# xingchensong/TouchNet

Hardware: AMD Instinct MI355X
Metric: audio+text tokens/sec/node (packed seq, full train step) + step MFU (higher is better)
Workload: dtype bf16

## Files before the change

### include/touchnet_amd.h

```cpp
#ifndef TOUCHNET_AMD_H_
#define TOUCHNET_AMD_H_

#ifdef __cplusplus
extern "C" {
#endif

const char* tn_version(void);

int tn_norm_bwd_workspace_floats(int rows, int H);
int tn_rmsnorm_fwd(const void* x, const void* res_in, const void* w, void* y, void* res_out, float* rstd,
                   int rows, int H, float eps, int dtype, void* stream);
int tn_rmsnorm_bwd(const void* dy, const void* h, const void* w, const float* rstd, const void* dres, void* dh,
                   void* dw, float* workspace, int rows, int H, int dtype, void* stream);

int tn_layernorm_fwd(const void* x, const void* res_in, const void* w, const void* b, void* y, void* res_out,
                     float* mean, float* rstd, int rows, int H, float eps, int dtype, void* stream);
int tn_layernorm_bwd(const void* dy, const void* h, const void* w, const float* mean, const float* rstd,
                     const void* dres, void* dh, void* dw, void* db, float* workspace, int rows, int H, int dtype,
                     void* stream);

int tn_swiglu_fwd(const void* gate, const void* up, void* out, long long n, int dtype, void* stream);
int tn_swiglu_bwd(const void* dout, const void* gate, const void* up, void* dgate, void* dup, long long n,
                  int dtype, void* stream);
int tn_swiglu_fwd_t(const void* gate, const void* up, void* out, void* out_t, int rows, int cols, void* stream);
// ... 79 lines not shown
int tn_transpose_bf16(const void* src, void* dst, int rows, int cols, long long src_ld, long long dst_ld,
                      void* stream);

long long tn_colsum_workspace_floats(int rows, int cols);
int tn_colsum_bf16(const void* x, void* out, float* ws, int rows, int cols, long long ld, void* stream);

int tn_pcm16_to_f32(const void* pcm_int16, float* out, long long n, void* stream);

int tn_bestrq_tokenize(const float* feat, const float* quantizer, const float* codebook, long long* codes, int T,
                       int F, int E, int V, void* stream);

int tn_pack_plan(const int* lens, int n, int B, int T, int skip_too_long, int* row, int* col, int* sent, int* batch,
                 int* counts, void* stream);
int tn_pack_fill(const int* row, const int* col, const int* sent, const int* batch, int which_batch, int n,
                 const int* ntok, const long long* tok_off, const long long* tokens, const int* alen,
                 const long long* feat_off, const float* feat_src, int F, int B, int T, long long bos, long long eos,
                 long long pad, long long* input_ids, long long* labels, long long* position_ids, long long* doc,
                 long long* sentence_lens, float* feats, int* nsent, void* stream);

int tn_gemm_bf16(const void* const* A, const void* const* B, const long long* lda, const long long* ldb, const int* K,
                 int nseg, int a_kmaj, int b_kmaj, void* C, void* Ct, const void* bias, int M, int N, long long ldc,
                 long long ldct, int accumulate, void* stream);
int tn_gemm_bf16_addend(const void* A, const void* B, long long lda, long long ldb, int K, int a_kmaj, int b_kmaj, void* C,
                        const void* bias, const void* addend, long long ldadd, int M, int N, long long ldc, void* stream);
int tn_gemm_bf16_splitk(const void* A, const void* B, long long lda, long long ldb, int K, int a_kmaj, int b_kmaj,
                        void* C, const void* bias, int M, int N, long long ldc, int accumulate, int splitk, int tail_only,
                        void* workspace, long long workspace_bytes, void* stream);
int tn_gemm_bf16_wgrad_f32(const void* A, const void* B, long long lda, long long ldb, int K, float* C, int M, int N,
                           long long ldc, int accumulate, int splitk, void* workspace, long long workspace_bytes,
                           void* stream);
int tn_gemm_bf16_wgrad_bias(const void* A, const void* B, long long lda, long long ldb, int K, void* C, void* bias_grad,
                            int M, int N, long long ldc, int accumulate, int c_f32, int splitk, void* workspace,
                            long long workspace_bytes, void* stream);
long long tn_gemm_grouped_workspace_bytes(const int* M, const int* N, const int* K, int ngrp);
int tn_gemm_bf16_grouped(const void* const* A, const void* const* B, const long long* lda, const long long* ldb,
                         const int* K, void* const* C, const long long* ldc, const int* M, const int* N, int ngrp,
                         int a_kmaj, int b_kmaj, int accumulate, int c_f32, void* workspace, long long workspace_bytes,
                         void* stream);
int tn_gemm_bf16_swiglu_fwd(const void* x, const void* wg, const void* wu, void* gate, void* up, void* act, int M, int I,
                            int K, long long ldx, long long ldw, long long ldc, void* stream);
int tn_gemm_bf16_swiglu_bwd(const void* dy, const void* wd, const void* gate, const void* up, void* dgate, void* dup,
                            int M, int I, int H, long long lddy, long long ldw, long long ld, void* stream);
int tn_gemm_bf16_gelu_fwd(const void* x, const void* w, const void* bias, void* pre, void* act, int M, int N, int K,
                          long long ldx, long long ldw, long long ldc, void* stream);
int tn_gemm_bf16_gelu_bwd(const void* dy, const void* w2, const void* pre, void* dpre, int M, int I, int H, long long lddy,
                          long long ldw, long long ld, void* stream);
int tn_gemm_bf16_rope(const void* x, const void* w, const void* bias, const void* cos_t, const void* sin_t, void* out, int M,
                      int N, int K, long long ldx, long long ldw, long long ldc, int head_dim, void* stream);
int tn_gemm_bf16_tn(const void* A, const void* B, void* C, void* Ct, const void* bias, int M, int N, int K,
                    long long lda, long long ldb, long long ldc, long long ldct, int accumulate, void* stream);

void tn_gemm_set_persistent(int on);
int tn_gemm_get_persistent(void);

long long tn_attn_decode_workspace_bytes(int B, int Nh, int Nkv, int D, int S_max);
int tn_attn_decode(const void* q, const void* k_new, const void* v_new, void* k_cache, void* v_cache, const int* cache_len,
                   void* o, void* workspace, int B, int Nh, int Nkv, int D, int S_max, float scale, void* stream);
int tn_greedy_step(const void* logits, int* hist, int* hist_len, int* cache_len, int* finished, int* n_unfinished, int B,
                   int V, int S_hist, float penalty, int ngram, int eos, int pad, int dtype, void* stream);
int tn_sample_step(const void* logits, int* hist, int* hist_len, int* cache_len, int* finished, int* n_unfinished,
                   const long long* row_key, const float* uniforms, int* n_kept, int B, int V, int S_hist, float penalty,
                   int do_sample, float temperature, int top_k, float top_p, unsigned long long seed, const int* eos_ids,
                   int n_eos, int pad, int dtype, void* stream);
int tn_kimi_text_step(const void* logits, int* hist, int* hist_len, int* cache_len, int* finished, int* n_unfinished,
                      const int* prompt_len, const void* embed, void* x_next, const long long* row_key,
                      const float* uniforms, int B, int V, int S_hist, int H, float penalty, int window, float temperature,
// ... 21 lines not shown
```

### touchnet_amd/_C.py

```python
from __future__ import annotations

import ctypes as C
import os

import torch

_HERE = os.path.dirname(os.path.abspath(__file__))
LIB_PATH = os.environ.get("TN_AMD_LIB") or os.path.join(_HERE, "_lib", "libtouchnet_amd.so")

_vp, _i, _f, _ll, _ull = C.c_void_p, C.c_int, C.c_float, C.c_longlong, C.c_ulonglong

PROTOTYPES = {
    "tn_version": [],
    "tn_norm_bwd_workspace_floats": [_i, _i],
    "tn_rmsnorm_fwd": [_vp, _vp, _vp, _vp, _vp, _vp, _i, _i, _f, _i, _vp],
    "tn_rmsnorm_bwd": [_vp, _vp, _vp, _vp, _vp, _vp, _vp, _vp, _i, _i, _i, _vp],
    "tn_layernorm_fwd": [_vp, _vp, _vp, _vp, _vp, _vp, _vp, _vp, _i, _i, _f, _i, _vp],
    "tn_layernorm_bwd": [_vp, _vp, _vp, _vp, _vp, _vp, _vp, _vp, _vp, _vp, _i, _i, _i, _vp],
    "tn_swiglu_fwd": [_vp, _vp, _vp, _ll, _i, _vp],
    "tn_swiglu_bwd": [_vp, _vp, _vp, _vp, _vp, _ll, _i, _vp],
    "tn_gelu_fwd": [_vp, _vp, _ll, _i, _vp],
    "tn_gelu_bwd": [_vp, _vp, _vp, _ll, _i, _vp],
    "tn_rope_table": [_vp, _vp, _vp, _vp, _i, _i, _f, _i, _vp],
    "tn_rope_apply": [_vp, _vp, _vp, _vp, _vp, _vp, _i, _i, _i, _i, _i, _i, _vp],
# ... 17 lines not shown
    "tn_log_mel": [_vp, _vp, _vp, _vp, _i, _i, _vp],
    "tn_audiofeat_stack": [_vp, _vp, _i, _i, _i, _i, _i, _vp],
    "tn_resample_polyphase": [_vp, _vp, _vp, _ll, _ll, _i, _i, _i, _vp],
    "tn_feat_augment": [_vp, _vp, _i, _i, _i, _vp, _i, _vp, _i, _vp, _i, _vp],
    "tn_sumsq_scratch_floats": [],
    "tn_sumsq": [_vp, _vp, _vp, _ll, _i, _vp],
    "tn_adamw_step": [_vp, _vp, _vp, _vp, _vp, _vp, _ll, _f, _f, _f, _f, _f, _f, _f, _f, _i, _vp],
    "tn_transpose_bf16": [_vp, _vp, _i, _i, _ll, _ll, _vp],
    "tn_swiglu_fwd_t": [_vp, _vp, _vp, _vp, _i, _i, _vp],
    "tn_swiglu_bwd_t": [_vp, _vp, _vp, _vp, _vp, _vp, _i, _i, _vp],
    "tn_colsum_workspace_floats": [_i, _i],
    "tn_colsum_bf16": [_vp, _vp, _vp, _i, _i, _ll, _vp],
    "tn_pcm16_to_f32": [_vp, _vp, _ll, _vp],
    "tn_bestrq_tokenize": [_vp, _vp, _vp, _vp, _i, _i, _i, _i, _vp],
    "tn_sumsq_multi_chunk": [],
    "tn_sumsq_multi": [_vp, _vp, _vp, _i, _ll, _vp, _vp, _i, _vp],
    "tn_adamw_multi_chunk": [],
    "tn_adamw_prepare": [_vp, _vp, _f, _f, _f, _vp],
    "tn_adamw_multi": [_vp, _vp, _vp, _vp, _vp, _vp, _vp, _i, _ll, _vp, _f, _f, _f, _f, _f, _i, _vp],
    "tn_adamw_multi_bounded": [_vp, _vp, _vp, _vp, _vp, _vp, _vp, _i, _ll, _vp, _f, _f, _f, _f, _f, _i, _i, _vp],
    "tn_pack_plan": [_vp, _i, _i, _i, _i, _vp, _vp, _vp, _vp, _vp, _vp],
    "tn_pack_fill": [_vp, _vp, _vp, _vp, _i, _i, _vp, _vp, _vp, _vp, _vp, _vp, _i, _i, _i, _ll, _ll, _ll, _vp, _vp, _vp,
                     _vp, _vp, _vp, _vp, _vp],
    "tn_gemm_bf16_tn": [_vp, _vp, _vp, _vp, _vp, _i, _i, _i, _ll, _ll, _ll, _ll, _i, _vp],
    "tn_gemm_bf16_addend": [_vp, _vp, _ll, _ll, _i, _i, _i, _vp, _vp, _vp, _ll, _i, _i, _ll, _vp],
    "tn_gemm_bf16_splitk": [_vp, _vp, _ll, _ll, _i, _i, _i, _vp, _vp, _i, _i, _ll, _i, _i, _i, _vp, _ll, _vp],
    "tn_gemm_bf16_wgrad_f32": [_vp, _vp, _ll, _ll, _i, _vp, _i, _i, _ll, _i, _i, _vp, _ll, _vp],
    "tn_gemm_bf16": [C.POINTER(_vp), C.POINTER(_vp), C.POINTER(_ll), C.POINTER(_ll), C.POINTER(_i), _i, _i, _i, _vp, _vp,
                     _vp, _i, _i, _ll, _ll, _i, _vp],
    "tn_gemm_grouped_workspace_bytes": [C.POINTER(_i), C.POINTER(_i), C.POINTER(_i), _i],
    "tn_gemm_bf16_grouped": [C.POINTER(_vp), C.POINTER(_vp), C.POINTER(_ll), C.POINTER(_ll), C.POINTER(_i), C.POINTER(_vp),
                             C.POINTER(_ll), C.POINTER(_i), C.POINTER(_i), _i, _i, _i, _i, _i, _vp, _ll, _vp],
    "tn_gemm_bf16_wgrad_bias": [_vp, _vp, _ll, _ll, _i, _vp, _vp, _i, _i, _ll, _i, _i, _i, _vp, _ll, _vp],
    "tn_gemm_bf16_rope": [_vp, _vp, _vp, _vp, _vp, _vp, _i, _i, _i, _ll, _ll, _ll, _i, _vp],
    "tn_gemm_bf16_gelu_fwd": [_vp, _vp, _vp, _vp, _vp, _i, _i, _i, _ll, _ll, _ll, _vp],
    "tn_gemm_bf16_gelu_bwd": [_vp, _vp, _vp, _vp, _i, _i, _i, _ll, _ll, _ll, _vp],
    "tn_gemm_bf16_swiglu_fwd": [_vp, _vp, _vp, _vp, _vp, _vp, _i, _i, _i, _ll, _ll, _ll, _vp],
    "tn_gemm_bf16_swiglu_bwd": [_vp, _vp, _vp, _vp, _vp, _vp, _i, _i, _i, _ll, _ll, _ll, _vp],
    "tn_gemm_set_persistent": [_i],
    "tn_gemm_get_persistent": [],
    "tn_attn_decode_workspace_bytes": [_i, _i, _i, _i, _i],
    "tn_attn_decode": [_vp, _vp, _vp, _vp, _vp, _vp, _vp, _vp, _i, _i, _i, _i, _i, _f, _vp],
    "tn_greedy_step": [_vp, _vp, _vp, _vp, _vp, _vp, _i, _i, _i, _f, _i, _i, _i, _i, _vp],
    "tn_sample_step": [_vp, _vp, _vp, _vp, _vp, _vp, _vp, _vp, _vp, _i, _i, _i, _f, _i, _f, _i, _f, _ull, _vp, _i, _i, _i,
                       _vp],
    "tn_kimi_text_step": [_vp] * 11 + [_i, _i, _i, _i, _f, _i, _f, _i, _ull, _i, _i, _i, _i, _vp],
    "tn_attn_decode_beam": [_vp, _vp, _vp, _vp, _vp, _vp, _vp, _vp, _vp, _i, _i, _i, _i, _i, _f, _vp],
    "tn_beam_step_workspace_bytes": [_i, _i],
    "tn_beam_step": [_vp] * 17 + [_i, _i, _i, _i, _i, _f, _i, _vp, _i, _i, _f, _i, _i, _vp],
    "tn_attn_block_causal_fwd": [_vp, _vp, _vp, _vp, _vp, _vp, _i, _i, _i, _i, _i, _f, _vp],
    "tn_vq_nearest": [_vp, _vp, _vp, _vp, _i, _i, _i, _vp],
}
_RESTYPE = {"tn_gemm_set_persistent": None, "tn_version": C.c_char_p, "tn_sumsq_multi_chunk": C.c_longlong, "tn_adamw_multi_chunk": C.c_longlong,
            "tn_colsum_workspace_floats": C.c_longlong, "tn_gemm_grouped_workspace_bytes": C.c_longlong,
            "tn_attn_decode_workspace_bytes": C.c_longlong, "tn_beam_step_workspace_bytes": C.c_longlong,
            "tn_philox4x32_10": None}

DEV_PROTOTYPES = {
    "tn_philox4x32_10": [_vp, _ull],
}

_lib = None


class KernelError(RuntimeError):
    pass
# ... 49 lines not shown
```

### touchnet_amd/csrc/gemm.hip

```cpp
#include <stdlib.h>

#include <type_traits>
#include <utility>

#include "common.h"

namespace tn {
namespace gemm {

constexpr int BM = 256, BN = 256;
constexpr int SLOT = 32768;
constexpr int LDS_BYTES = 5 * SLOT;
constexpr int NT = 512;
constexpr int MAXSEG = 3;

typedef __attribute__((address_space(3))) void* lds_ptr_t;
typedef __attribute__((ext_vector_type(2))) uint32_t u32x2_t;
typedef __attribute__((ext_vector_type(4))) uint32_t u32x4_t;

struct Seg {
  const bf16_t* A;
  const bf16_t* B;
  long long lda, ldb;
  int K;
// ... 7 lines not shown
  int start;
  int stages;
};

constexpr int EPI_PLAIN = 0, EPI_GROUPED = 1, EPI_SWIGLU_FWD = 2, EPI_SWIGLU_BWD = 3, EPI_BIASG = 4, EPI_ROPE = 5;
constexpr int EPI_GELU_FWD = 6, EPI_GELU_BWD = 7;

struct Params {
  Seg seg[MAXSEG];
  int nseg;
  int M, N;
  bf16_t* C;
  bf16_t* Ct;
  const bf16_t* bias;
  long long ldc, ldct;
  int accumulate;
  const bf16_t* addend;
  long long ldadd;
  int nbm, nbn;
  int stages;
  int splitk, kchunk;
  float* ws;
  int tile0, ntiles;
  int c_f32;
  Grp grp[MAXSEG];
  int ngrp;
  bf16_t* C2;
  bf16_t* C3;
  const bf16_t* E1;
  const bf16_t* E2;
  long long lde;
  bf16_t* bias_out;
  float* bias_ws;
  const bf16_t* rope_cos;
  const bf16_t* rope_sin;
  int rope_d;
};

__device__ __forceinline__ void tile_of_block(int bid, int nbm, int nbn, int& tm, int& tn) {
  const int total = nbm * nbn;
  const int xcd = bid & 7, local = bid >> 3;
  const int q = total >> 3, r = total & 7;
  const int vid = (xcd < r ? xcd * (q + 1) : r * (q + 1) + (xcd - r) * q) + local;
  constexpr int GM = 8;
  const int per_group = GM * nbn;
  const int g = vid / per_group, w = vid - g * per_group;
  const int gm = min(GM, nbm - g * GM);
  tm = g * GM + w % gm;
  tn = w / gm;
}

typedef f32x16_t Acc[4][2];

constexpr int kPieceB[4] = {0, 2, 4, 6}, kPieceA[4] = {14, 18, 22, 26};
static_assert(kPieceB[3] < kPieceA[0], "every B piece is issued before the first A piece");

template <bool IS_A> constexpr int piece_at(int pos) {
  for (int i = 0; i < 4; ++i)
    if ((IS_A ? kPieceA[i] : kPieceB[i]) == pos) return i;
  return -1;
}
constexpr int early_piece_count() {
  int n = 0;
  for (int i = 0; i < 4; ++i) n += (kPieceB[i] < 8) + (kPieceA[i] < 8);
  return n;
}
// ... 235 lines not shown
    auto zero_acc = [&]() {
#pragma unroll
      for (int i = 0; i < 4; ++i)
#pragma unroll
        for (int j = 0; j < 2; ++j)
#pragma unroll
          for (int r = 0; r < 16; ++r) acc[i][j][r] = 0.f;
    };
    zero_acc();

    Frags<AK, 4> ae, ao;
    Frags<BK, 2> be, bo;

#define TN_PIN() __builtin_amdgcn_sched_barrier(0)
    auto read_frag = [&](auto QC, auto FC, int sa, int sb, Frags<AK, 4>& a, Frags<BK, 2>& b) {
      constexpr int Q = decltype(QC)::value, F = decltype(FC)::value;
      if constexpr (F < 2) rb.template read<Q, F>(smem, sb * SLOT, b);
      else ra.template read<Q, F - 2>(smem, sa * SLOT, a);
    };
    auto read_all = [&](auto QC, int sa, int sb, Frags<AK, 4>& a, Frags<BK, 2>& b) {
      read_frag(QC, std::integral_constant<int, 0>{}, sa, sb, a, b);
      read_frag(QC, std::integral_constant<int, 1>{}, sa, sb, a, b);
      read_frag(QC, std::integral_constant<int, 2>{}, sa, sb, a, b);
      read_frag(QC, std::integral_constant<int, 3>{}, sa, sb, a, b);
      read_frag(QC, std::integral_constant<int, 4>{}, sa, sb, a, b);
      read_frag(QC, std::integral_constant<int, 5>{}, sa, sb, a, b);
    };
    auto mma = [&](const Frags<AK, 4>& a, const Frags<BK, 2>& b, int i, int j) {
      acc[i][j] = __builtin_amdgcn_mfma_f32_32x32x16_bf16(b.v[j], a.v[i], acc[i][j], 0, 0, 0);
    };

    float bsum = 0.f;
    bool bias_on = false;
    auto bias_accum = [&](const Frags<AK, 4>& a) {
      auto add = [&](const bf16x8_t& v) {
        const u32x4_t w = __builtin_bit_cast(u32x4_t, v);
        bsum += ((__uint_as_float(w.x << 16) + __uint_as_float(w.x & 0xffff0000u)) +
                 (__uint_as_float(w.y << 16) + __uint_as_float(w.y & 0xffff0000u))) +
                ((__uint_as_float(w.z << 16) + __uint_as_float(w.z & 0xffff0000u)) +
                 (__uint_as_float(w.w << 16) + __uint_as_float(w.w & 0xffff0000u)));
      };
      if (wc == 0) add(a.v[0]);
      else if (wc == 1) add(a.v[1]);
      else if (wc == 2) add(a.v[2]);
      else add(a.v[3]);
    };

    auto quarter = [&](auto NQC, auto P0C, const Frags<AK, 4>& ca, const Frags<BK, 2>& cb, Frags<AK, 4>& na,
                       Frags<BK, 2>& nb, int nsa, int nsb, int dst_b, int dst_a) {
      constexpr int P0 = decltype(P0C)::value;
      if constexpr (EPI == EPI_BIASG) {
        if (bias_on) bias_accum(ca);
        TN_PIN();
      }
      auto step = [&](auto MC) {
        constexpr int m = decltype(MC)::value;
        mma(ca, cb, m >> 1, m & 1);
        TN_PIN();
        if constexpr (m < 6) {
          read_frag(NQC, std::integral_constant<int, m>{}, nsa, nsb, na, nb);
          TN_PIN();
        }
        constexpr int pb = P0 < 0 ? -1 : piece_at<false>(P0 + m);
        constexpr int pa = P0 < 0 ? -1 : piece_at<true>(P0 + m);
        if constexpr (pb >= 0) {
          piece_b(dst_b, pb);
// ... 32 lines not shown
      one(std::integral_constant<int, 1>{});
      one(std::integral_constant<int, 2>{});
      one(std::integral_constant<int, 3>{});
      one(std::integral_constant<int, 4>{});
      one(std::integral_constant<int, 5>{});
      one(std::integral_constant<int, 6>{});
      one(std::integral_constant<int, 7>{});
    };
    auto next = [](int s, int d) { s += d; return s >= 5 ? s - 5 : s; };
    using I0 = std::integral_constant<int, 0>;
    using I1 = std::integral_constant<int, 1>;
    using I2 = std::integral_constant<int, 2>;
    using I3 = std::integral_constant<int, 3>;
    using NONE = std::integral_constant<int, -1>;

#pragma unroll
    for (int q = 0; q < 4; ++q) piece_a(0, q);
    adv_a();
#pragma unroll
    for (int q = 0; q < 4; ++q) piece_b(1, q);
    adv_b();
#pragma unroll
    for (int q = 0; q < 4; ++q) piece_a(2, q);
    adv_a();
    early_pieces(3, 4);
    asm volatile("s_waitcnt vmcnt(%0)" ::"n"(4 + early_piece_count()) : "memory");
    __builtin_amdgcn_s_barrier();
    int sa = 0, sb = 1;
    int pa = 4, pb = 3;

    auto trip = [&](auto LASTC) {
      constexpr bool LAST = decltype(LASTC)::value;
      const int sa1 = next(sa, 2), sb1 = next(sb, 2);
      __builtin_amdgcn_s_setprio(1);
      quarter(I1{}, std::integral_constant<int, 8>{}, ae, be, ao, bo, sa, sb, pb, pa);
      wait_frags(ao, bo);
      TN_PIN();
      quarter(I2{}, std::integral_constant<int, 16>{}, ao, bo, ae, be, sa, sb, pb, pa);
      wait_frags(ae, be);
      TN_PIN();
      quarter(I3{}, std::integral_constant<int, 24>{}, ae, be, ao, bo, sa, sb, pb, pa);
      __builtin_amdgcn_s_setprio(0);
      wait_frags(ao, bo);
      __builtin_amdgcn_s_waitcnt(0xc07f);
      asm volatile("s_waitcnt vmcnt(4)" ::: "memory");
      __builtin_amdgcn_s_barrier();
      __builtin_amdgcn_s_setprio(1);
      if constexpr (!LAST) {
        quarter(I0{}, I0{}, ao, bo, ae, be, sa1, sb1, sa, sb);
        __builtin_amdgcn_s_setprio(0);
        wait_frags(ae, be);
        TN_PIN();
      } else {
        if constexpr (EPI == EPI_BIASG) {
          if (bias_on) bias_accum(ao);
        }
#pragma unroll
        for (int m = 0; m < 8; ++m) mma(ao, bo, m >> 1, m & 1);
        __builtin_amdgcn_s_setprio(0);
      }
      pb = sa;
      pa = sb;
      sa = sa1;
      sb = sb1;
    };

    const int np_all = SPLITK ? p.kchunk : p.stages;
    for (int kc = 0; kc < mine; ++kc) {
      int np = np_all;
      if constexpr (EPI == EPI_BIASG) {
        int m0_, n0_, g_;
        origin_g(kc, m0_, n0_, g_);
        bias_on = n0_ == 0;
        bsum = 0.f;
      }
      if constexpr (EPI == EPI_GROUPED) {
        int m0_, n0_, g_;
        origin_g(kc, m0_, n0_, g_);
        np = p.grp[g_].stages;
      }
      read_all(I0{}, sa, sb, ae, be);
      wait_frags(ae, be);
      TN_PIN();
      for (int t = 1; t < np; ++t) trip(std::false_type{});
      trip(std::true_type{});
      int m0, n0, grp;
      origin_g(kc, m0, n0, grp);
      if constexpr (EPI == EPI_BIASG) {
        if (bias_on) {
          const float tot = bsum + __shfl_xor(bsum, 32, 64);
          const int m = m0 + wr * 128 + wc * 32 + (lane & 31);
          if (lane < 32) {
            if constexpr (SPLITK) {
              p.bias_ws[(long long)split_of(kc) * (p.nbm * BM) + m] = tot;
            } else if (m < p.M) {
              p.bias_out[m] = f2bf(tot);
            }
          }
        }
      }
      if constexpr (SPLITK) {
        const int u = bid + kc * G, sp = u / tiles;
        epilogue_ws(p, acc, sp * tiles + (u - sp * tiles), wr * 128, wc * 64, lane);
      } else if constexpr (OUT_F32) {
        if constexpr (EPI == EPI_GROUPED) {
          const Out o = {p.grp[grp].C, p.grp[grp].ldc, p.grp[grp].M, p.grp[grp].N};
          epilogue_f32(p, o, acc, m0 + wr * 128, n0 + wc * 64, lane);
        } else {
          const Out o = {p.C, p.ldc, p.M, p.N};
          epilogue_f32(p, o, acc, m0 + wr * 128, n0 + wc * 64, lane);
        }
      } else if constexpr (EPI == EPI_GROUPED) {
        const Out o = {p.grp[grp].C, p.grp[grp].ldc, p.grp[grp].M, p.grp[grp].N};
        epilogue(p, o, acc, smem + (wave < 4 ? pb : pa) * SLOT + (wave & 3) * 8192, m0 + wr * 128, n0 + wc * 64, lane);
      } else {
        const Out o = {p.C, p.ldc, p.M, p.N};
        epilogue(p, o, acc, smem + (wave < 4 ? pb : pa) * SLOT + (wave & 3) * 8192, m0 + wr * 128, n0 + wc * 64, lane);
      }
      zero_acc();
      __builtin_amdgcn_s_waitcnt(0xc07f);
      __builtin_amdgcn_s_barrier();
      asm volatile("" : "+v"(lane));
      ra = Reader<AK, 4>(lane, wr * 128);
      rb = Reader<BK, 2>(lane, wc * 64);
      sA.set_voff(wave, lane);
      sB.set_voff(wave, lane);
      early_pieces(pb, pa);
// ... 765 lines not shown
    float* d = reinterpret_cast<float*>(C) + (long long)m * ldc + n;
    float4 x = make_float4(a[0], a[1], a[2], a[3]), y = make_float4(a[4], a[5], a[6], a[7]);
    if (accumulate) {
      const float4 ox = *reinterpret_cast<const float4*>(d), oy = *reinterpret_cast<const float4*>(d + 4);
      x.x += ox.x; x.y += ox.y; x.z += ox.z; x.w += ox.w;
      y.x += oy.x; y.y += oy.y; y.z += oy.z; y.w += oy.w;
    }
    *reinterpret_cast<float4*>(d) = x;
    *reinterpret_cast<float4*>(d + 4) = y;
    return;
  }
  bf16_t* dst = C + (long long)m * ldc + n;
  if (bias != nullptr) {
    Vec16<bf16_t> b;
    float fb[8];
    b.load(bias + n);
    b.unpack(fb);
#pragma unroll
    for (int e = 0; e < 8; ++e) a[e] += fb[e];
  }
  if (accumulate) {
    Vec16<bf16_t> o;
    float fo[8];
    o.load(dst);
    o.unpack(fo);
#pragma unroll
    for (int e = 0; e < 8; ++e) a[e] += fo[e];
  }
  Vec16<bf16_t> out;
  out.pack(a);
  out.store(dst);
}

template <bool AK, bool BK, bool HAS_CT>
static int launch(dim3 grid, hipStream_t st, const Params& p) {
  constexpr bool WGRAD = AK && BK && !HAS_CT;
  auto reduce = [&](const float* bias_ws, bf16_t* bias_out) {
    hipLaunchKernelGGL(splitk_reduce_kernel, dim3((unsigned)p.ntiles * 32u), dim3(256), 0, st, p.ws, p.splitk, p.M, p.N,
                       p.nbm, p.nbn, p.tile0, p.ntiles, p.C, p.ldc, p.bias, p.accumulate, p.c_f32, bias_ws, bias_out);
  };
  if (p.bias_out != nullptr) {
    if constexpr (WGRAD) {
      if (p.splitk > 1) {
        hipLaunchKernelGGL((gemm_kernel<true, true, false, true, false, EPI_BIASG>), grid, dim3(NT), 0, st, p);
        reduce(p.bias_ws, p.bias_out);
      } else if (p.c_f32) {
        hipLaunchKernelGGL((gemm_kernel<true, true, false, false, true, EPI_BIASG>), grid, dim3(NT), 0, st, p);
      } else {
        hipLaunchKernelGGL((gemm_kernel<true, true, false, false, false, EPI_BIASG>), grid, dim3(NT), 0, st, p);
      }
    } else {
      return -1;
    }
  } else if (p.splitk > 1) {
    if constexpr (!HAS_CT) {
      hipLaunchKernelGGL((gemm_kernel<AK, BK, false, true>), grid, dim3(NT), 0, st, p);
      reduce(nullptr, nullptr);
    } else {
      return -1;
    }
  } else if (p.c_f32) {
    if constexpr (WGRAD) {
      hipLaunchKernelGGL((gemm_kernel<true, true, false, false, true>), grid, dim3(NT), 0, st, p);
    } else {
      return -1;
    }
  } else if constexpr (!AK && !HAS_CT) {
    hipLaunchKernelGGL((gemm16_kernel<AK, BK>), grid, dim3(NT), 0, st, p);
  } else {
    hipLaunchKernelGGL((gemm_kernel<AK, BK, HAS_CT>), grid, dim3(NT), 0, st, p);
  }
  return 0;
}

}
}

extern "C" {

static int g_persistent = 1;
void tn_gemm_set_persistent(int on) { g_persistent = on ? 1 : 0; }
int tn_gemm_get_persistent(void) { return g_persistent; }

// ... 64 lines not shown
  }
  for (int s = nseg; s < MAXSEG; ++s) p.seg[s] = p.seg[0];
  if (Ct != nullptr && ((M % 8) || (ldct % 8) || ldct < M || ((uintptr_t)Ct & 15))) return TN_EINVAL;
  if (Ct != nullptr && accumulate) return TN_EINVAL;
  p.nseg = nseg;
  p.M = M;
  p.N = N;
  p.C = (tn::bf16_t*)C;
  p.Ct = (tn::bf16_t*)Ct;
  p.bias = (const tn::bf16_t*)bias;
  p.ldc = ldc;
  p.ldct = ldct;
  p.accumulate = accumulate;
  p.addend = (const tn::bf16_t*)addend;
  p.ldadd = ldadd;
  p.nbm = (M + BM - 1) / BM;
  p.nbn = (N + BN - 1) / BN;
  p.splitk = 1;
  p.kchunk = 0;
  p.ws = nullptr;
  p.tile0 = 0;
  p.ntiles = p.nbm * p.nbn;
  p.c_f32 = c_f32;
  const int ncu = num_cus();
  int main_tiles = 0;
  if (splitk > 1) {
    if (nseg != 1 || Ct != nullptr) return TN_EINVAL;
    if (!(a_kmaj && b_kmaj) && (p.stages % splitk) != 0) return TN_EINVAL;
    if (tail_only) {
      main_tiles = p.ntiles / ncu * ncu;
      if (main_tiles <= 0 || main_tiles >= p.ntiles) return TN_EINVAL;
    }
    const long long slabs = (long long)splitk * (p.ntiles - main_tiles) * BM * BN;
    if (workspace == nullptr || ((uintptr_t)workspace & 15) ||
        workspace_bytes < (slabs + (bias_grad ? (long long)splitk * p.nbm * BM : 0)) * (long long)sizeof(float))
      return TN_EINVAL;
    p.splitk = splitk;
    p.kchunk = (p.stages + splitk - 1) / splitk;
    p.ws = (float*)workspace;
    p.bias_ws = bias_grad ? (float*)workspace + slabs : nullptr;
  }
  p.bias_out = (tn::bf16_t*)bias_grad;
  const bool persist = persistent_now();
  hipStream_t st = (hipStream_t)stream;
  int rc = 0;
#define TN_MODE(AKM, BKM, GRID, PRM) \
  rc |= (Ct != nullptr) ? launch<AKM, BKM, true>(GRID, st, PRM) : launch<AKM, BKM, false>(GRID, st, PRM)
#define TN_LAUNCH(GRID, PRM)                                                               \
  if (!a_kmaj && !b_kmaj) TN_MODE(false, false, GRID, PRM);                                \
  else if (!a_kmaj && b_kmaj) TN_MODE(false, true, GRID, PRM);                             \
  else if (a_kmaj && b_kmaj) TN_MODE(true, true, GRID, PRM);                               \
  else return TN_EINVAL
  if (main_tiles > 0) {
    Params pm = p;
    pm.splitk = 1;
    pm.ntiles = main_tiles;
    const dim3 gm(ncu);
    TN_LAUNCH(gm, pm);
    p.tile0 = main_tiles;
    p.ntiles -= main_tiles;
  }
  {
    const int units = p.ntiles * p.splitk;
    const dim3 grid(persist && units > ncu ? ncu : units);
    TN_LAUNCH(grid, p);
  }
#undef TN_LAUNCH
#undef TN_MODE
  if (rc != 0) return TN_EINVAL;
  TN_LAUNCH_CHECK();
  return TN_OK;
}

// ... 183 lines not shown
    return TN_EINVAL;
  Params p;
  clear_params(p);
  p.seg[0].A = (const tn::bf16_t*)dy;
  p.seg[0].B = (const tn::bf16_t*)wd;
  p.seg[0].lda = lddy;
  p.seg[0].ldb = ldw;
  p.seg[0].K = H;
  p.seg[1] = p.seg[2] = p.seg[0];
  p.stages = H / 64;
  p.M = M;
  p.N = I;
  p.C = (tn::bf16_t*)dgate;
  p.C2 = (tn::bf16_t*)dup;
  p.E1 = (const tn::bf16_t*)gate;
  p.E2 = (const tn::bf16_t*)up;
  p.ldc = p.lde = ld;
  p.nbm = (M + BM - 1) / BM;
  p.nbn = (I + BN - 1) / BN;
  p.ntiles = p.nbm * p.nbn;
  const int ncu = num_cus();
  const dim3 grid(persistent_now() && p.ntiles > ncu ? ncu : p.ntiles);
  hipLaunchKernelGGL((gemm16_kernel<false, true, EPI_SWIGLU_BWD>), grid, dim3(NT), 0, (hipStream_t)stream, p);
  TN_LAUNCH_CHECK();
  return TN_OK;
}

int tn_gemm_bf16_wgrad_bias(const void* A, const void* B, long long lda, long long ldb, int K, void* C, void* bias_grad,
                            int M, int N, long long ldc, int accumulate, int c_f32, int splitk, void* workspace,
                            long long workspace_bytes, void* stream) {
  if (bias_grad == nullptr) return TN_EINVAL;
  return gemm_launch(&A, &B, &lda, &ldb, &K, 1, 1, 1, C, nullptr, nullptr, M, N, ldc, 0, accumulate,
                     splitk > 1 ? splitk : 1, 0, workspace, workspace_bytes, stream, c_f32, bias_grad);
}

int tn_gemm_bf16_rope(const void* x, const void* w, const void* bias, const void* cos_t, const void* sin_t, void* out, int M,
                      int N, int K, long long ldx, long long ldw, long long ldc, int head_dim, void* stream) {
  using namespace tn::gemm;
  if (M <= 0 || N <= 0 || K <= 0 || (K % 64) || (ldx % 8) || (ldw % 8) || (ldc % 8) || ldc < N) return TN_EINVAL;
  if (ldx < K || ldw < K) return TN_EINVAL;
  if (!((head_dim == 128 && N % 256 == 0) || (head_dim == 64 && N % 64 == 0))) return TN_EINVAL;
  if (((uintptr_t)x | (uintptr_t)w | (uintptr_t)out) & 15) return TN_EINVAL;
  if (((uintptr_t)cos_t | (uintptr_t)sin_t | (uintptr_t)bias) & 7) return TN_EINVAL;
  if (cos_t == nullptr || sin_t == nullptr) return TN_EINVAL;
  if ((long long)288 * ldx * 2 >= 0x7fffffffLL || (long long)288 * ldw * 2 >= 0x7fffffffLL) return TN_EINVAL;
  Params p;
  clear_params(p);
  p.seg[0].A = (const tn::bf16_t*)x;
  p.seg[0].B = (const tn::bf16_t*)w;
  p.seg[0].lda = ldx;
  p.seg[0].ldb = ldw;
  p.seg[0].K = K;
  p.seg[1] = p.seg[2] = p.seg[0];
  p.stages = K / 64;
  p.M = M;
  p.N = N;
  p.C = (tn::bf16_t*)out;
  p.bias = (const tn::bf16_t*)bias;
  p.ldc = ldc;
  p.rope_cos = (const tn::bf16_t*)cos_t;
  p.rope_sin = (const tn::bf16_t*)sin_t;
  p.rope_d = head_dim;
  p.nbm = (M + BM - 1) / BM;
  p.nbn = (N + BN - 1) / BN;
  p.ntiles = p.nbm * p.nbn;
  const int ncu = num_cus();
// ... 78 lines not shown
```

### touchnet_amd/functional.py

```python
from __future__ import annotations

import math
import os
from dataclasses import dataclass
from typing import Optional

import torch

from . import _C
from . import library as L

_cur = _C.stream
_p = _C.ptr


def _c(t: torch.Tensor) -> torch.Tensor:
    return t if t.is_contiguous() else t.contiguous()


def rms_norm(x, weight, eps, residual=None):
    y, h, _ = L.rmsnorm_fwd(x, residual, weight, float(eps))
    return (y, h) if residual is not None else y


# ... 352 lines not shown
    return out


def gemm(segs, a_kmaj: bool = False, b_kmaj: bool = False, bias: Optional[torch.Tensor] = None,
         out: Optional[torch.Tensor] = None, accumulate: bool = False,
         out_t: Optional[torch.Tensor] = None, bias_grad: Optional[torch.Tensor] = None,
         addend: Optional[torch.Tensor] = None) -> torch.Tensor:
    if not 1 <= len(segs) <= 3:
        raise _C.KernelError("gemm: 1..3 segments")
    for a, b in segs:
        if a.dim() != 2 or b.dim() != 2 or a.dtype != torch.bfloat16 or b.dtype != torch.bfloat16:
            raise _C.KernelError("gemm: 2-D bf16 operands only")
        if a.stride(1) != 1 or b.stride(1) != 1:
            raise _C.KernelError("gemm: operands need contiguous rows")
    a0, b0 = segs[0]
    M = a0.shape[1] if a_kmaj else a0.shape[0]
    N = b0.shape[1] if b_kmaj else b0.shape[0]
    Ks = []
    for a, b in segs:
        Ka, Ma = (a.shape[0], a.shape[1]) if a_kmaj else (a.shape[1], a.shape[0])
        Kb, Nb = (b.shape[0], b.shape[1]) if b_kmaj else (b.shape[1], b.shape[0])
        if Ka != Kb or Ma != M or Nb != N:
            raise _C.KernelError(f"gemm: segment shapes disagree: a {tuple(a.shape)} b {tuple(b.shape)}")
        Ks.append(Ka)
    if out is None:
        if accumulate:
            raise _C.KernelError("gemm: accumulate needs `out`")
        out = torch.empty(M, N, dtype=torch.bfloat16, device=a0.device)
    if out.dtype == torch.float32:
        if not (a_kmaj and b_kmaj and len(segs) == 1 and bias is None and out_t is None):
            raise _C.KernelError("gemm: fp32 output exists for the single-segment weight-gradient mode only")
        if out.stride(1) != 1 or tuple(out.shape) != (M, N) or not a0.is_cuda:
            raise _C.KernelError("gemm: bad fp32 `out`")
        split = split_k(M, N, Ks[0], True, True) if SPLIT_K else 1
        ws = None
        if split > 1:
            ws = torch.empty(split * (((M + 255) // 256) * ((N + 255) // 256) * 65536 + (M + 255) // 256 * 256),
                             dtype=torch.float32, device=a0.device)
        if bias_grad is not None:
            _check_bias_grad(bias_grad, M, a0)
            _C.check(_C.lib().tn_gemm_bf16_wgrad_bias(_p(a0), _p(b0), a0.stride(0), b0.stride(0), Ks[0], _p(out), _p(bias_grad),
                                                      M, N, out.stride(0), int(accumulate), 1, split, _p(ws),
                                                      ws.numel() * 4 if ws is not None else 0, _cur()),
                     "tn_gemm_bf16_wgrad_bias")
            return out
        _C.check(_C.lib().tn_gemm_bf16_wgrad_f32(_p(a0), _p(b0), a0.stride(0), b0.stride(0), Ks[0], _p(out), M, N,
                                                 out.stride(0), int(accumulate), split, _p(ws),
                                                 ws.numel() * 4 if ws is not None else 0, _cur()), "tn_gemm_bf16_wgrad_f32")
        return out
    if out.stride(1) != 1 or tuple(out.shape) != (M, N) or out.dtype != torch.bfloat16:
        raise _C.KernelError("gemm: bad `out`")
    if bias is not None:
        bias = _c(bias).to(torch.bfloat16)
    n = len(segs)
    if not a0.is_cuda:
        raise _C.KernelError("touchnet_amd kernels need device (HIP) tensors; got a CPU tensor")
    if addend is not None:
        if (n != 1 or accumulate or out_t is not None or bias_grad is not None or addend.dtype != torch.bfloat16
                or tuple(addend.shape) != (M, N) or addend.stride(1) != 1 or addend.data_ptr() == out.data_ptr()):
            raise _C.KernelError("gemm: addend needs one segment, a bf16 [M, N] matrix with contiguous rows that is not `out`")
        _C.check(_C.lib().tn_gemm_bf16_addend(_p(a0), _p(b0), a0.stride(0), b0.stride(0), Ks[0], int(a_kmaj), int(b_kmaj),
                                              _p(out), _p(bias), _p(addend), addend.stride(0), M, N, out.stride(0), _cur()),
                 "tn_gemm_bf16_addend")
        return out
    split = 1
    if bias_grad is not None:
        if not (a_kmaj and b_kmaj and n == 1 and bias is None and out_t is None):
            raise _C.KernelError("gemm: bias_grad exists for the single-segment weight-gradient mode only")
        _check_bias_grad(bias_grad, M, a0)
        split = split_k(M, N, Ks[0], True, True) if SPLIT_K else 1
        ws = None
        if split > 1:
            ws = torch.empty(split * (((M + 255) // 256) * ((N + 255) // 256) * 65536 + (M + 255) // 256 * 256),
                             dtype=torch.float32, device=a0.device)
        _C.check(_C.lib().tn_gemm_bf16_wgrad_bias(_p(a0), _p(b0), a0.stride(0), b0.stride(0), Ks[0], _p(out), _p(bias_grad), M,
                                                  N, out.stride(0), int(accumulate), 0, split, _p(ws),
                                                  ws.numel() * 4 if ws is not None else 0, _cur()), "tn_gemm_bf16_wgrad_bias")
        return out
    if n == 1 and out_t is None and SPLIT_K:
        split = split_k(M, N, Ks[0], a_kmaj, b_kmaj)
    if split > 1:
        tiles = ((M + 255) // 256) * ((N + 255) // 256)
        ws = torch.empty(split * tiles * 65536, dtype=torch.float32, device=a0.device)
        _C.check(_C.lib().tn_gemm_bf16_splitk(_p(a0), _p(b0), a0.stride(0), b0.stride(0), Ks[0], int(a_kmaj), int(b_kmaj),
                                              _p(out), _p(bias), M, N, out.stride(0), int(accumulate), split, 0,
                                              _p(ws), ws.numel() * 4, _cur()), "tn_gemm_bf16_splitk")
        return out
    import ctypes as C
    Ap = (C.c_void_p * n)(*[a.data_ptr() for a, _ in segs])
    Bp = (C.c_void_p * n)(*[b.data_ptr() for _, b in segs])
    la = (C.c_longlong * n)(*[a.stride(0) for a, _ in segs])
    lb = (C.c_longlong * n)(*[b.stride(0) for _, b in segs])
    Kc = (C.c_int * n)(*Ks)
    _C.check(_C.lib().tn_gemm_bf16(Ap, Bp, la, lb, Kc, n, int(a_kmaj), int(b_kmaj), _p(out), _p(out_t), _p(bias), M, N,
                                   out.stride(0), out_t.stride(0) if out_t is not None else 0, int(accumulate),
                                   _cur()), "tn_gemm_bf16")
    return out


def _check_bias_grad(bias_grad, M, like):
    if (bias_grad.dtype != torch.bfloat16 or bias_grad.dim() != 1 or bias_grad.numel() != M or not bias_grad.is_contiguous()
            or bias_grad.device != like.device):
        raise _C.KernelError("gemm: bias_grad must be a contiguous bf16 [M] device vector")


def gemm_grouped_wgrad(pairs, outs=None, accumulate: bool = False):
    import ctypes as C
    n = len(pairs)
    if not 1 <= n <= 3:
        raise _C.KernelError("gemm_grouped_wgrad: 1..3 products")
    for a, b in pairs:
        if (a.dim() != 2 or b.dim() != 2 or a.dtype != torch.bfloat16 or b.dtype != torch.bfloat16 or a.stride(1) != 1
                or b.stride(1) != 1 or a.shape[0] != b.shape[0] or not a.is_cuda):
            raise _C.KernelError("gemm_grouped_wgrad: pairs of 2-D bf16 device matrices [K, M] / [K, N] with contiguous rows")
    if outs is None:
        if accumulate:
            raise _C.KernelError("gemm_grouped_wgrad: accumulate needs `outs`")
        outs = [torch.empty(a.shape[1], b.shape[1], dtype=torch.bfloat16, device=a.device) for a, b in pairs]
    f32 = outs[0].dtype == torch.float32
    for o, (a, b) in zip(outs, pairs):
        if (o.dtype != outs[0].dtype or o.dtype not in (torch.float32, torch.bfloat16) or o.stride(1) != 1
                or tuple(o.shape) != (a.shape[1], b.shape[1])):
            raise _C.KernelError("gemm_grouped_wgrad: bad `outs`")
    Ms = (C.c_int * n)(*[a.shape[1] for a, _ in pairs])
    Ns = (C.c_int * n)(*[b.shape[1] for _, b in pairs])
    Ks = (C.c_int * n)(*[a.shape[0] for a, _ in pairs])
    need = int(_C.lib().tn_gemm_grouped_workspace_bytes(Ms, Ns, Ks, n))
    ws = torch.empty(need // 4, dtype=torch.float32, device=outs[0].device) if need > 0 else None
    Ap = (C.c_void_p * n)(*[a.data_ptr() for a, _ in pairs])
    Bp = (C.c_void_p * n)(*[b.data_ptr() for _, b in pairs])
# ... 819 lines not shown
```

Measured before the change: 23010.

## Pick wgrad split-K with a cost model and slice bias-grad across N tiles

Adds a host-side cost model (tn_gemm_wgrad_parts) that picks the split-K factor for weight-gradient GEMMs from tile count, K stages and CU count, replacing the previous split_k heuristic. The bias-gradient reduction is also spread across all N-tile columns: each tile writes its partial row sum to a sliced workspace, and a new bias_finish kernel sums them. Before, only tiles at n0==0 did that work. This is meant to fill more CUs on small-tile wgrad GEMMs and to balance the bias work. The cost is larger workspaces, an extra small kernel launch, and hand-tuned timing constants that may not fit every shape.

```diff
diff --git a/include/touchnet_amd.h b/include/touchnet_amd.h
--- a/include/touchnet_amd.h
+++ b/include/touchnet_amd.h
@@ -135,6 +135,7 @@
 int tn_gemm_bf16_wgrad_bias(const void* A, const void* B, long long lda, long long ldb, int K, void* C, void* bias_grad,
                             int M, int N, long long ldc, int accumulate, int c_f32, int splitk, void* workspace,
                             long long workspace_bytes, void* stream);
+int tn_gemm_wgrad_parts(int M, int N, int K);
 long long tn_gemm_grouped_workspace_bytes(const int* M, const int* N, const int* K, int ngrp);
 int tn_gemm_bf16_grouped(const void* const* A, const void* const* B, const long long* lda, const long long* ldb,
                          const int* K, void* const* C, const long long* ldc, const int* M, const int* N, int ngrp,
diff --git a/touchnet_amd/_C.py b/touchnet_amd/_C.py
--- a/touchnet_amd/_C.py
+++ b/touchnet_amd/_C.py
@@ -73,6 +73,7 @@
     "tn_gemm_bf16_grouped": [C.POINTER(_vp), C.POINTER(_vp), C.POINTER(_ll), C.POINTER(_ll), C.POINTER(_i), C.POINTER(_vp),
                              C.POINTER(_ll), C.POINTER(_i), C.POINTER(_i), _i, _i, _i, _i, _i, _vp, _ll, _vp],
     "tn_gemm_bf16_wgrad_bias": [_vp, _vp, _ll, _ll, _i, _vp, _vp, _i, _i, _ll, _i, _i, _i, _vp, _ll, _vp],
+    "tn_gemm_wgrad_parts": [_i, _i, _i],
     "tn_gemm_bf16_rope": [_vp, _vp, _vp, _vp, _vp, _vp, _i, _i, _i, _ll, _ll, _ll, _i, _vp],
     "tn_gemm_bf16_gelu_fwd": [_vp, _vp, _vp, _vp, _vp, _i, _i, _i, _ll, _ll, _ll, _vp],
     "tn_gemm_bf16_gelu_bwd": [_vp, _vp, _vp, _vp, _i, _i, _i, _ll, _ll, _ll, _vp],
diff --git a/touchnet_amd/csrc/gemm.hip b/touchnet_amd/csrc/gemm.hip
--- a/touchnet_amd/csrc/gemm.hip
+++ b/touchnet_amd/csrc/gemm.hip
@@ -63,6 +63,7 @@
   long long lde;
   bf16_t* bias_out;
   float* bias_ws;
+  int bias_sliced;
   const bf16_t* rope_cos;
   const bf16_t* rope_sin;
   int rope_d;
@@ -364,6 +365,7 @@
 
     float bsum = 0.f;
     bool bias_on = false;
+    int bias_next = 0, bias_per = 1;
     auto bias_accum = [&](const Frags<AK, 4>& a) {
       auto add = [&](const bf16x8_t& v) {
         const u32x4_t w = __builtin_bit_cast(u32x4_t, v);
@@ -462,6 +464,10 @@
     auto trip = [&](auto LASTC) {
       constexpr bool LAST = decltype(LASTC)::value;
       const int sa1 = next(sa, 2), sb1 = next(sb, 2);
+      if constexpr (EPI == EPI_BIASG) {
+        bias_on = bias_next == 0;
+        bias_next = bias_on ? bias_per - 1 : bias_next - 1;
+      }
       __builtin_amdgcn_s_setprio(1);
       quarter(I1{}, std::integral_constant<int, 8>{}, ae, be, ao, bo, sa, sb, pb, pa);
       wait_frags(ao, bo);
@@ -501,7 +507,9 @@
       if constexpr (EPI == EPI_BIASG) {
         int m0_, n0_, g_;
         origin_g(kc, m0_, n0_, g_);
-        bias_on = n0_ == 0;
+        const int tn_ = n0_ / BN;
+        bias_per = p.bias_sliced ? p.nbn : 1;
+        bias_next = (p.bias_sliced || tn_ == 0) ? tn_ : 0x7fffffff;
         bsum = 0.f;
       }
       if constexpr (EPI == EPI_GROUPED) {
@@ -517,12 +525,15 @@
       int m0, n0, grp;
       origin_g(kc, m0, n0, grp);
       if constexpr (EPI == EPI_BIASG) {
-        if (bias_on) {
+        if (p.bias_sliced || n0 == 0) {
           const float tot = bsum + __shfl_xor(bsum, 32, 64);
           const int m = m0 + wr * 128 + wc * 32 + (lane & 31);
           if (lane < 32) {
-            if constexpr (SPLITK) {
-              p.bias_ws[(long long)split_of(kc) * (p.nbm * BM) + m] = tot;
+            const int sp = SPLITK ? split_of(kc) : 0;
+            if (p.bias_sliced) {
+              p.bias_ws[((long long)sp * p.nbn + n0 / BN) * (p.nbm * BM) + m] = tot;
+            } else if constexpr (SPLITK) {
+              p.bias_ws[(long long)sp * (p.nbm * BM) + m] = tot;
             } else if (m < p.M) {
               p.bias_out[m] = f2bf(tot);
             }
@@ -1354,6 +1365,8 @@
   out.store(dst);
 }
 
+void bias_finish(const float* partials, int rows, int pitch, int M, bf16_t* bias_out, hipStream_t st);
+
 template <bool AK, bool BK, bool HAS_CT>
 static int launch(dim3 grid, hipStream_t st, const Params& p) {
   constexpr bool WGRAD = AK && BK && !HAS_CT;
@@ -1365,12 +1378,14 @@
     if constexpr (WGRAD) {
       if (p.splitk > 1) {
         hipLaunchKernelGGL((gemm_kernel<true, true, false, true, false, EPI_BIASG>), grid, dim3(NT), 0, st, p);
-        reduce(p.bias_ws, p.bias_out);
+        if (p.bias_sliced) reduce(nullptr, nullptr);
+        else reduce(p.bias_ws, p.bias_out);
       } else if (p.c_f32) {
         hipLaunchKernelGGL((gemm_kernel<true, true, false, false, true, EPI_BIASG>), grid, dim3(NT), 0, st, p);
       } else {
         hipLaunchKernelGGL((gemm_kernel<true, true, false, false, false, EPI_BIASG>), grid, dim3(NT), 0, st, p);
       }
+      if (p.bias_sliced) bias_finish(p.bias_ws, p.splitk * p.nbn, p.nbm * BM, p.M, p.bias_out, st);
     } else {
       return -1;
     }
@@ -1501,13 +1516,19 @@
       if (main_tiles <= 0 || main_tiles >= p.ntiles) return TN_EINVAL;
     }
     const long long slabs = (long long)splitk * (p.ntiles - main_tiles) * BM * BN;
+    const long long rows = (long long)splitk * p.nbm * BM;
     if (workspace == nullptr || ((uintptr_t)workspace & 15) ||
-        workspace_bytes < (slabs + (bias_grad ? (long long)splitk * p.nbm * BM : 0)) * (long long)sizeof(float))
+        workspace_bytes < (slabs + (bias_grad ? rows : 0)) * (long long)sizeof(float))
       return TN_EINVAL;
     p.splitk = splitk;
     p.kchunk = (p.stages + splitk - 1) / splitk;
     p.ws = (float*)workspace;
     p.bias_ws = bias_grad ? (float*)workspace + slabs : nullptr;
+    p.bias_sliced = bias_grad != nullptr && workspace_bytes >= (slabs + rows * p.nbn) * (long long)sizeof(float);
+  } else if (bias_grad != nullptr && workspace != nullptr && !((uintptr_t)workspace & 15) &&
+             workspace_bytes >= (long long)p.nbn * p.nbm * BM * (long long)sizeof(float)) {
+    p.bias_ws = (float*)workspace;
+    p.bias_sliced = 1;
   }
   p.bias_out = (tn::bf16_t*)bias_grad;
   const bool persist = persistent_now();
@@ -1757,6 +1778,34 @@
   if (bias_grad == nullptr) return TN_EINVAL;
   return gemm_launch(&A, &B, &lda, &ldb, &K, 1, 1, 1, C, nullptr, nullptr, M, N, ldc, 0, accumulate,
                      splitk > 1 ? splitk : 1, 0, workspace, workspace_bytes, stream, c_f32, bias_grad);
+}
+
+constexpr double kStageUs = 0.845, kStageBusyUs = 0.586, kUnitUs = 8.4, kReduceUs = 0.7, kReduceUsPerMB = 0.386;
+constexpr double kSecondRoundGain = 0.05;
+constexpr long long kWgradWsCap = 256ll << 20;
+int tn_gemm_wgrad_parts(int M, int N, int K) {
+  using namespace tn::gemm;
+  if (M <= 0 || N <= 0 || K <= 0) return 1;
+  const int ncu = num_cus();
+  const long long tiles = (long long)((M + BM - 1) / BM) * ((N + BN - 1) / BN);
+  const int stages = (K + 63) / 64;
+  if (tiles * 2 > ncu || stages < 16) return 1;
+  int best[2] = {1, 0};
+  double best_us[2] = {0., 0.};
+  for (int parts = 1; parts <= stages / 8 && tiles * parts <= 2 * ncu; ++parts) {
+    const long long bytes = parts > 1 ? tiles * parts * (long long)(BM * BN * sizeof(float)) : 0;
+    if (bytes > kWgradWsCap) break;
+    const int kchunk = (stages + parts - 1) / parts;
+    double us = parts > 1 ? kReduceUs + (double)bytes * kReduceUsPerMB / (1 << 20) : 0.;
+    for (long long left = tiles * parts; left > 0; left -= ncu)
+      us += kchunk * (kStageUs + kStageBusyUs * (double)(left < ncu ? left : ncu) / ncu) + kUnitUs;
+    const int r = tiles * parts > ncu;
+    if (best[r] == 0 || parts == 1 || us < best_us[r]) {
+      best[r] = parts;
+      best_us[r] = us;
+    }
+  }
+  return best[1] != 0 && best_us[1] < (1. - kSecondRoundGain) * best_us[0] ? best[1] : best[0];
 }
 
 int tn_gemm_bf16_rope(const void* x, const void* w, const void* bias, const void* cos_t, const void* sin_t, void* out, int M,
diff --git a/touchnet_amd/csrc/gemm_bias_finish.hip b/touchnet_amd/csrc/gemm_bias_finish.hip
--- /dev/null
+++ b/touchnet_amd/csrc/gemm_bias_finish.hip
@@ -0,0 +1,21 @@
+#include "common.h"
+
+namespace tn {
+namespace gemm {
+
+__global__ __launch_bounds__(256) void bias_finish_kernel(const float* __restrict__ partials, int rows, int pitch, int M,
+                                                          bf16_t* __restrict__ bias_out) {
+  const int m = blockIdx.x * 256 + threadIdx.x;
+  if (m >= M) return;
+  float s = 0.f;
+  for (int r = 0; r < rows; ++r) s += partials[(long long)r * pitch + m];
+  bias_out[m] = f2bf(s);
+}
+
+void bias_finish(const float* partials, int rows, int pitch, int M, bf16_t* bias_out, hipStream_t st) {
+  hipLaunchKernelGGL(bias_finish_kernel, dim3((unsigned)(M + 255) / 256u), dim3(256), 0, st, partials, rows, pitch, M,
+                     bias_out);
+}
+
+}
+}
diff --git a/touchnet_amd/functional.py b/touchnet_amd/functional.py
--- a/touchnet_amd/functional.py
+++ b/touchnet_amd/functional.py
@@ -408,11 +408,8 @@
             raise _C.KernelError("gemm: fp32 output exists for the single-segment weight-gradient mode only")
         if out.stride(1) != 1 or tuple(out.shape) != (M, N) or not a0.is_cuda:
             raise _C.KernelError("gemm: bad fp32 `out`")
-        split = split_k(M, N, Ks[0], True, True) if SPLIT_K else 1
-        ws = None
-        if split > 1:
-            ws = torch.empty(split * (((M + 255) // 256) * ((N + 255) // 256) * 65536 + (M + 255) // 256 * 256),
-                             dtype=torch.float32, device=a0.device)
+        split = wgrad_parts(M, N, Ks[0])
+        ws = _wgrad_workspace(M, N, split, bias_grad is not None, a0.device)
         if bias_grad is not None:
             _check_bias_grad(bias_grad, M, a0)
             _C.check(_C.lib().tn_gemm_bf16_wgrad_bias(_p(a0), _p(b0), a0.stride(0), b0.stride(0), Ks[0], _p(out), _p(bias_grad),
@@ -444,17 +441,14 @@
         if not (a_kmaj and b_kmaj and n == 1 and bias is None and out_t is None):
             raise _C.KernelError("gemm: bias_grad exists for the single-segment weight-gradient mode only")
         _check_bias_grad(bias_grad, M, a0)
-        split = split_k(M, N, Ks[0], True, True) if SPLIT_K else 1
-        ws = None
-        if split > 1:
-            ws = torch.empty(split * (((M + 255) // 256) * ((N + 255) // 256) * 65536 + (M + 255) // 256 * 256),
-                             dtype=torch.float32, device=a0.device)
+        split = wgrad_parts(M, N, Ks[0])
+        ws = _wgrad_workspace(M, N, split, True, a0.device)
         _C.check(_C.lib().tn_gemm_bf16_wgrad_bias(_p(a0), _p(b0), a0.stride(0), b0.stride(0), Ks[0], _p(out), _p(bias_grad), M,
                                                   N, out.stride(0), int(accumulate), 0, split, _p(ws),
                                                   ws.numel() * 4 if ws is not None else 0, _cur()), "tn_gemm_bf16_wgrad_bias")
         return out
     if n == 1 and out_t is None and SPLIT_K:
-        split = split_k(M, N, Ks[0], a_kmaj, b_kmaj)
+        split = wgrad_parts(M, N, Ks[0]) if a_kmaj and b_kmaj else split_k(M, N, Ks[0], a_kmaj, b_kmaj)
     if split > 1:
         tiles = ((M + 255) // 256) * ((N + 255) // 256)
         ws = torch.empty(split * tiles * 65536, dtype=torch.float32, device=a0.device)
@@ -472,6 +466,16 @@
                                    out.stride(0), out_t.stride(0) if out_t is not None else 0, int(accumulate),
                                    _cur()), "tn_gemm_bf16")
     return out
+
+
+def wgrad_parts(M: int, N: int, K: int) -> int:
+    return int(_C.lib().tn_gemm_wgrad_parts(M, N, K)) if SPLIT_K else 1
+
+
+def _wgrad_workspace(M: int, N: int, split: int, bias: bool, device) -> Optional[torch.Tensor]:
+    nbm, nbn = (M + 255) // 256, (N + 255) // 256
+    floats = (split * nbm * nbn * 65536 if split > 1 else 0) + (split * nbn * nbm * 256 if bias else 0)
+    return torch.empty(floats, dtype=torch.float32, device=device) if floats else None
 
 
 def _check_bias_grad(bias_grad, M, like):
```

Result: no change. 22970 (-0.2%).
